# robertknight/rten

Hardware: NVIDIA H100
Metric: resnet50_fp32_inferences_per_sec (higher is better)
Workload: dtype f32(tf32 mma, explicit opt-in)

## Files before the change

rten_b200/csrc/umma_gemm.cu:

```cuda
#include <cuda.h>
#include <cuda_runtime.h>

#include <algorithm>
#include <array>
#include <cmath>
#include <vector>
#include <cmath>
#include <cstdint>
#include <cstdio>
#include <cstdlib>

#include "math.cuh"
#include "ptx.cuh"
#include "rowops.h"
#include "umma_gemm.h"
#include "umma_kernel.cuh"

namespace rtb {

typedef CUresult (*EncodeTiledFn)(CUtensorMap*, CUtensorMapDataType, cuuint32_t, void*, const cuuint64_t*,
                                  const cuuint64_t*, const cuuint32_t*, const cuuint32_t*, CUtensorMapInterleave,
                                  CUtensorMapSwizzle, CUtensorMapL2promotion, CUtensorMapFloatOOBfill);

static EncodeTiledFn get_encode(rten_ctx* ctx) {
    if (!ctx->encode_tiled) {
        void* fn = nullptr;
        cudaDriverEntryPointQueryResult qres;
        if (cudaGetDriverEntryPoint("cuTensorMapEncodeTiled", &fn, cudaEnableDefault, &qres) != cudaSuccess ||
            qres != cudaDriverEntryPointSuccess)
            return nullptr;
        ctx->encode_tiled = fn;
    }
    return reinterpret_cast<EncodeTiledFn>(ctx->encode_tiled);
}

bool tma_compatible(const OperandDesc& od, int esize, int rank) {
    if (reinterpret_cast<uintptr_t>(od.base) & 15) return false;
    if (od.strides[0] != 1) return false;
    for (int i = 1; i < rank; i++) {
        if (od.dims[i] > 1) {
            if ((od.strides[i] * esize) % 16 != 0) return false;
            if (od.strides[i] * esize >= (1ll << 40)) return false;
        }
    }
    for (int i = 0; i < rank; i++)
        if (od.dims[i] < 1 || od.dims[i] > 0xFFFFFFFFll) return false;
    return true;
}

bool encode_map(rten_ctx* ctx, CUtensorMap* map, const OperandDesc& od, int esize, bool is_f32,
                const uint32_t box[4], const uint32_t estr[4]) {
    EncodeTiledFn enc = get_encode(ctx);
    if (!enc) return false;
    cuuint64_t dims[4];
    cuuint64_t strides[3];
    cuuint32_t b[4], es[4];
    for (int i = 0; i < 4; i++) {
        dims[i] = (cuuint64_t)od.dims[i];
        b[i] = box[i];
        es[i] = estr[i];
    }
    for (int i = 1; i < 4; i++) {
        long long s = od.strides[i] * esize;
        if (s == 0 || od.dims[i] == 1) s = 16;
        strides[i - 1] = (cuuint64_t)s;
    }
    CUresult r = enc(map, is_f32 ? CU_TENSOR_MAP_DATA_TYPE_FLOAT32 : CU_TENSOR_MAP_DATA_TYPE_UINT8, 4,
                     const_cast<void*>(od.base), dims, strides, b, es, CU_TENSOR_MAP_INTERLEAVE_NONE,
                     CU_TENSOR_MAP_SWIZZLE_128B, CU_TENSOR_MAP_L2_PROMOTION_L2_256B,
                     CU_TENSOR_MAP_FLOAT_OOB_FILL_NONE);
    return r == CUDA_SUCCESS;
}

static void pick_conv_tile(const ConvGeom& g, int& tw, int& th, int& tb) {
    double best = -1.0;
    tw = th = tb = 1;
    for (int w = 1; w <= std::min(g.OW, 128); w++) {
        if (w * g.sx > 256) break;
        for (int h = 1; h <= std::min(g.OH, 128 / w); h++) {
            if (h * g.sy > 256) break;
            int b = std::min(g.B, 128 / (w * h));
            if (b < 1) continue;
            long long tiles = (long long)((g.OW + w - 1) / w) * ((g.OH + h - 1) / h) * ((g.B + b - 1) / b);
            double eff = (double)g.B * g.OH * g.OW / ((double)tiles * 128.0);
            if (eff > best + 1e-9 || (eff > best - 1e-9 && w > tw)) {
                best = eff;
                tw = w;
                th = h;
                tb = b;
            }
        }
    }
}

struct Plan {
    int bn = 32, splitk = 1, nbuf = 1;
};

struct Prepared {
    KParams p;
    uint32_t abox[4], aes[4], bbox_k;
    uint32_t a_rows;
    long long batch;
    OperandDesc od, ord;
    uint32_t dbox[4];
    int tma_store, res_tma;
    int wide;
    int step;
    int esize, kelems;
};

constexpr int SK_CNT_INTS = 1 << 16;
static int smem_budget_for(int n_stg) { return 227 * 1024 - SMEM_FIXED_BYTES - n_stg * STG_BYTES; }
static int wide_stages(int stage_bytes) { return std::min(MAX_STAGES, (227 * 1024 - WIDE_SMEM_FIXED_BYTES) / stage_bytes); }
static bool is_wide(int bn) { return bn > ACC_STRIDE; }

static Epi pick_epilogue(const GemmLaunch& L, int tma_store, int res_tma, int splitk) {
    const EpilogueDesc& e = L.epi;
    auto aligned = [](const void* ptr) { return (reinterpret_cast<uintptr_t>(ptr) & 15) == 0; };
    bool fast = tma_store && (L.N % 32) == 0 && !getenv("RTEN_B200_NO_FAST") && e.bias_kind != 2 &&
                (e.r == nullptr || res_tma) && (e.bias_kind != 1 || aligned(e.bias));
    if (L.kind == 1)
        fast = fast && (!(e.za || e.za8) || aligned(e.colsum)) && (!e.zb || e.zb_len == 1 || (e.zb_len == L.N && aligned(e.zb))) &&
               (!e.scale || e.scale_len == 1 || (e.scale_len == L.N && aligned(e.scale)));
    if (!fast) return Epi::Generic;
    const bool gelu = e.act > 1;
    if (!getenv("RTEN_B200_NO_PLAIN") && e.act <= 3) {
        if (L.kind == 0 && e.alpha == 1.0f && !e.range && (e.r == nullptr || e.r_scale == 1.0f))
            return gelu ? Epi::PlainF32Gelu : Epi::PlainF32;
        if (L.kind == 1 && e.scale && !e.za && !e.zb && (e.scale_len == 1 || e.scale_len == L.N) && splitk == 1 &&
            (!e.za8 || e.colsum))
            return gelu ? Epi::PlainI8Gelu : Epi::PlainI8;
    }
    return gelu ? Epi::FastGelu : Epi::Fast;
}

static const char* epi_name(Epi v) {
    static const char* const names[] = {"Generic", "Fast", "FastGelu", "PlainF32", "PlainF32Gelu", "PlainI8", "PlainI8Gelu"};
    return names[(int)v];
}

static bool is_plain_f32(Epi v) { return v == Epi::PlainF32 || v == Epi::PlainF32Gelu; }

struct PlanShape {
    long long tiles_n, units_m, tiles, units;
    int kb_per, stage_bytes, stages, n_stg;
};

static bool plan_shape(const Prepared& q, const Plan& pl, PlanShape& ps) {
    const KParams& p = q.p;
    if (is_wide(pl.bn)) {
        if ((pl.bn != 128 && pl.bn != 256) || !q.wide || pl.splitk != 1) return false;
        if (pl.bn == 256 && q.p.epi.act > 1) return false;
    } else if (pl.bn < 16 || pl.bn % 32 || pl.bn % q.step) {
        return false;
    }
    if (pl.nbuf < (q.res_tma ? 2 : 1) || pl.nbuf > 4) return false;
    ps.tiles_n = (p.N + pl.bn - 1) / pl.bn;
    ps.units_m = p.tiles_m;
    ps.tiles = ps.units_m * ps.tiles_n * q.batch;
    ps.units = ps.tiles * pl.splitk;
    if (ps.units > 0x7FFFFFFFll) return false;
    ps.kb_per = (p.k_blocks + pl.splitk - 1) / pl.splitk;
    if (pl.splitk > 1) {
        if (pl.bn % 32 || (long long)(pl.splitk - 1) * ps.kb_per >= p.k_blocks) return false;
        if (ps.tiles * 2 > SK_CNT_INTS) return false;
    }
    ps.n_stg = 2 * pl.nbuf;
    ps.stage_bytes = A_STAGE_BYTES + pl.bn * KBYTES;
    ps.stages = is_wide(pl.bn) ? wide_stages(ps.stage_bytes) : std::min(MAX_STAGES, smem_budget_for(ps.n_stg) / ps.stage_bytes);
    if (ps.stages < 2) return false;
    return true;
}

static double plan_cost(const Prepared& q, const Plan& pl, const PlanShape& ps, int num_sms) {
    const double active = (double)std::min<long long>(ps.units, num_sms);
    const double waves = std::ceil((double)ps.units / num_sms);
    const double bw = std::min(64.0, 7400.0 / active);
    const double mmas = 4.0;
    const double t_kb = std::max(mmas * std::max(42.0, (double)pl.bn), ps.stage_bytes / bw);
    double t_stage = std::max(t_kb, 320.0 + mmas * 42.0);
    t_stage = std::max(t_stage, 2300.0 / ps.stages);
    const double mainloop = ps.kb_per * t_stage;
    const double epi = is_wide(pl.bn) ? (pl.bn / 32.0) * 400.0 + 600.0 : (pl.bn / 32.0) * 350.0 / 2.0 + 600.0;
    double unit = (is_wide(pl.bn) ? mainloop + epi : std::max(mainloop, epi)) + 1500.0;
    double cost = waves * unit + 2500.0;
    if (pl.splitk > 1) cost += epi * (1.0 + 0.25 * pl.splitk) + 1500.0;

    return cost;
}

static void enumerate_plans(const Prepared& q, int num_sms, std::vector<std::pair<double, Plan>>& out) {
    const KParams& p = q.p;
    const int nmax = (p.N + q.step - 1) / q.step * q.step;
    static const int splits[] = {1, 2, 3, 4, 5, 6, 8, 10, 12, 16};
    for (int bn : {32, 64, 128, 256}) {
        if (bn > nmax && bn != 32) break;
        for (int sk : splits) {
            Plan pl;
            pl.bn = bn;
            pl.splitk = sk;
            if (sk > 1 && p.k_blocks / sk < 4) continue;
            const int kb_per = (p.k_blocks + sk - 1) / sk;
            pl.nbuf = (q.res_tma || kb_per < 24) ? 2 : 1;
            PlanShape ps;
            if (is_wide(bn)) {
                pl.nbuf = 2;
            } else if (pl.nbuf == 2 && !getenv("RTEN_B200_NO_NBUF3")) {
                PlanShape ps2;
                const bool ok2 = plan_shape(q, pl, ps2);
                pl.nbuf = 3;
                if (!plan_shape(q, pl, ps) || (ps.stages < 3 && !(ok2 && ps.stages == ps2.stages))) pl.nbuf = 2;
            }
            if (!plan_shape(q, pl, ps)) continue;
            if (sk > 1 && ps.tiles >= 2 * num_sms) continue;
            if (ps.stages < 2) continue;
            out.emplace_back(plan_cost(q, pl, ps, num_sms), pl);
        }
    }
    std::sort(out.begin(), out.end(), [](const std::pair<double, Plan>& x, const std::pair<double, Plan>& y) {
        return x.first < y.first;
    });
}

static rten_status prepare_launch(rten_ctx* ctx, const GemmLaunch& L, Prepared& q) {
    const int esize = L.kind == 0 ? 4 : 1;
    const int kelems = KBYTES / esize;
    if (!tma_compatible(L.a, esize, 4) || !tma_compatible(L.b, esize, 4)) return RTEN_ERR_UNSUPPORTED_VALUE;
    if (L.M <= 0 || L.N <= 0 || L.K <= 0) return RTEN_ERR_UNSUPPORTED_VALUE;
    q.esize = esize;
    q.kelems = kelems;
    KParams& p = q.p;
    memset(&p, 0, sizeof(p));
    p.M = L.M;
    p.N = L.N;
    p.K = L.K;
    p.z0 = L.z0;
    p.z1 = L.z1;
    p.kelems = kelems;
    p.conv = L.conv;
    p.epi = L.epi;
    p.c_blocks = 1;
    p.kw = 1;
    for (int i = 0; i < 4; i++) q.aes[i] = 1;
    if (L.conv) {
        const ConvGeom& g = L.g;
        pick_conv_tile(g, p.tw, p.th, p.tb);
        p.tiles_x = (g.OW + p.tw - 1) / p.tw;
        p.tiles_y = (g.OH + p.th - 1) / p.th;
        int tiles_b = (g.B + p.tb - 1) / p.tb;
        p.tiles_m = p.tiles_x * p.tiles_y * tiles_b;
        p.OH = g.OH;
        p.OW = g.OW;
        p.Bn = g.B;
        p.sy = g.sy;
        p.sx = g.sx;
        p.dy = g.dy;
        p.dx = g.dx;
        p.pt = g.pt;
        p.pl = g.pl;
        p.kw = g.kw;
        p.c_blocks = (g.C + kelems - 1) / kelems;
        p.k_blocks = g.kh * g.kw * p.c_blocks;
        p.z0 = p.z1 = 1;
        q.abox[0] = kelems;
        q.abox[1] = p.tw * g.sx;
        q.abox[2] = p.th * g.sy;
        q.abox[3] = p.tb;
        q.aes[1] = g.sx;
        q.aes[2] = g.sy;
        q.a_rows = p.tw * p.th * p.tb;
        q.batch = 1;
    } else {
        p.tiles_m = (L.M + BM - 1) / BM;
        p.k_blocks = (L.K + kelems - 1) / kelems;
        q.abox[0] = kelems;
        q.abox[1] = BM;
        q.abox[2] = 1;
        q.abox[3] = 1;
        q.a_rows = BM;
        q.batch = (long long)L.z0 * L.z1;
        p.a_bcast0 = (L.a.dims[2] == 1 && L.z0 > 1) ? 1 : 0;
        p.a_bcast1 = (L.a.dims[3] == 1 && L.z1 > 1) ? 1 : 0;
        p.b_bcast0 = (L.b.dims[2] == 1 && L.z0 > 1) ? 1 : 0;
        p.b_bcast1 = (L.b.dims[3] == 1 && L.z1 > 1) ? 1 : 0;
    }
    OperandDesc& od = q.od;
    OperandDesc& ord = q.ord;
    q.dbox[0] = 32;
    q.dbox[1] = q.dbox[2] = q.dbox[3] = 1;
    const EpilogueDesc& e = L.epi;
    od.base = e.d;
    od.dims[0] = L.N;
    od.strides[0] = 1;
    if (L.conv) {
        od.dims[1] = L.g.OW;
        od.dims[2] = L.g.OH;
        od.dims[3] = L.g.B;
        od.strides[1] = e.s_z1;
        od.strides[2] = e.s_row;
        od.strides[3] = e.s_z0;
        q.dbox[1] = p.tw;
        q.dbox[2] = p.th;
        q.dbox[3] = p.tb;
    } else {
        od.dims[1] = L.M;
        od.dims[2] = L.z0;
        od.dims[3] = L.z1;
        od.strides[1] = e.s_row;
        od.strides[2] = e.s_z0;
        od.strides[3] = e.s_z1;
        q.dbox[1] = BM;
    }
    q.tma_store = (e.s_col == 1 && L.N >= 4 && tma_compatible(od, 4, 4)) ? 1 : 0;
    if (getenv("RTEN_B200_NO_TMA_STORE")) q.tma_store = 0;
    ord = od;
    ord.base = e.r;
    if (L.conv) {
        ord.strides[1] = e.r_z1;
        ord.strides[2] = e.r_row;
        ord.strides[3] = e.r_z0;
    } else {
        ord.strides[1] = e.r_row;
        ord.strides[2] = e.r_z0;
        ord.strides[3] = e.r_z1;
    }
    q.res_tma = (q.tma_store && (L.kind == 0 || e.scale) && e.r && e.r_col == 1 && (L.N % 32) == 0 &&
                 (e.bias_kind != 1 || (reinterpret_cast<uintptr_t>(e.bias) & 15) == 0) && tma_compatible(ord, 4, 4))
                    ? 1
                    : 0;
    for (int i = 1; i < 4; i++)
        if (ord.dims[i] > 1 && ord.strides[i] == 0) q.res_tma = 0;
    if (getenv("RTEN_B200_NO_RES_TMA")) q.res_tma = 0;
    p.res_tx_bytes = q.a_rows * KBYTES;
    q.step = q.tma_store ? 32 : 16;
    q.wide = is_plain_f32(pick_epilogue(L, q.tma_store, q.res_tma, 1)) && !getenv("RTEN_B200_NO_WIDE");
    return RTEN_OK;
}

static size_t splitk_ws_bytes(const PlanShape& ps, const Plan& pl) {
    return pl.splitk > 1 ? (size_t)ps.tiles * pl.splitk * (pl.bn / 32) * 4096 * 4 : 0;
}

static rten_status ensure_splitk_counters(rten_ctx* ctx) {
    if (!ctx->sk_counters) {
        cudaError_t ce = cudaMalloc(&ctx->sk_counters, SK_CNT_INTS * sizeof(int));
        if (ce != cudaSuccess) return fail_cuda(ctx, ce, "split-K counters");
        ce = cudaMemset(ctx->sk_counters, 0, SK_CNT_INTS * sizeof(int));
        if (ce != cudaSuccess) return fail_cuda(ctx, ce, "split-K counters");
    }
    return RTEN_OK;
}

static rten_status launch_plan(rten_ctx* ctx, const GemmLaunch& L, const Prepared& q, const Plan& pl, bool verbose,
                               void* ws = nullptr) {
    PlanShape ps;
    if (!plan_shape(q, pl, ps)) return RTEN_ERR_UNSUPPORTED_VALUE;
    KParams p = q.p;
    p.bn = pl.bn;
    p.splitk = pl.splitk;
    p.nbuf = pl.nbuf;
    p.tma_store = q.tma_store;
    p.res_tma = q.res_tma ? 1 : 0;
    p.kb_per = ps.kb_per;
    p.tiles_n = (int)ps.tiles_n;
    p.tiles_total = (int)ps.tiles;
    p.units_total = (int)ps.units;
    p.d_tiles_n.set(p.tiles_n);
    p.d_tiles_m.set(p.tiles_m);
    p.d_z0.set(p.z0);
    p.d_tiles_x.set(p.conv ? p.tiles_x : 1);
    p.d_tiles_y.set(p.conv ? p.tiles_y : 1);
    p.d_tiles_total.set(p.tiles_total);
    p.d_c_blocks.set(p.c_blocks);
    p.d_kw.set(p.kw);
    p.d_tw.set(p.conv ? p.tw : 1);
    p.d_th.set(p.conv ? p.th : 1);
    p.stage_bytes = ps.stage_bytes;
    p.tx_bytes = q.a_rows * KBYTES + p.bn * KBYTES;
    p.stages = ps.stages;
    p.sgn = L.kind == 0 ? 0 : (L.a_signed ? 1 : 0) | (L.b_signed ? 2 : 0);
    if (p.splitk > 1) {
        RTB_TRY(ensure_splitk_counters(ctx));
        if (!ws) RTB_TRY(temp_alloc(ctx, splitk_ws_bytes(ps, pl), &ws));
        p.sk_ws = reinterpret_cast<uint32_t*>(ws);
        p.sk_cnt = reinterpret_cast<int*>(ctx->sk_counters);
    }

    uint32_t bbox[4] = {(uint32_t)q.kelems, (uint32_t)p.bn, 1, 1}, bes[4] = {1, 1, 1, 1}, des[4] = {1, 1, 1, 1};
    CUtensorMap map_a, map_b;
    if (!encode_map(ctx, &map_a, L.a, q.esize, L.kind == 0, q.abox, q.aes)) return RTEN_ERR_UNSUPPORTED_VALUE;
    if (!encode_map(ctx, &map_b, L.b, q.esize, L.kind == 0, bbox, bes)) return RTEN_ERR_UNSUPPORTED_VALUE;
    CUtensorMap map_d = map_a, map_r = map_a, map_a2 = map_a;
    p.x3_cb = L.x3_cb;
    if (L.x3_cb && !encode_map(ctx, &map_a2, L.a_lo, q.esize, true, q.abox, q.aes)) return RTEN_ERR_UNSUPPORTED_VALUE;
    if (p.tma_store && !encode_map(ctx, &map_d, q.od, 4, true, q.dbox, des)) {
        p.tma_store = 0;
        p.res_tma = 0;
        map_d = map_a;
    }
    if (p.res_tma && !encode_map(ctx, &map_r, q.ord, 4, true, q.dbox, des)) {
        p.res_tma = 0;
        map_r = map_a;
    }
    const Epi epi = pick_epilogue(L, p.tma_store, p.res_tma, p.splitk);
    if (epi == Epi::Generic && (L.kind == 1 || L.epi.act > 1)) p.res_tma = 0;

    if (verbose)
        fprintf(stderr, "[umma_gemm] kind=%d conv=%d M=%d N=%d K=%d kb=%d tiles_m=%d bn=%d splitk=%d units=%d stages=%d tma_store=%d res_tma=%d nbuf=%d box=%dx%dx%d epi=%s\n",
                L.kind, L.conv, L.M, L.N, L.K, p.k_blocks, p.tiles_m, p.bn, p.splitk, p.units_total, p.stages, p.tma_store,
                p.res_tma, p.nbuf, p.tw, p.th, p.tb, epi_name(epi));
    if (is_wide(p.bn) && !is_plain_f32(epi)) return RTEN_ERR_UNSUPPORTED_VALUE;
    const size_t smem_bytes = (size_t)p.stages * p.stage_bytes +
                              (is_wide(p.bn) ? WIDE_SMEM_FIXED_BYTES : ps.n_stg * STG_BYTES + SMEM_FIXED_BYTES);
    using Kernel = void (*)(CUtensorMap, CUtensorMap, CUtensorMap, CUtensorMap, CUtensorMap, KParams);
    static const Kernel narrow[2][7] = {
        {umma_gemm_kernel<0, Epi::Generic>, umma_gemm_kernel<0, Epi::Fast>, umma_gemm_kernel<0, Epi::FastGelu>,
         umma_gemm_kernel<0, Epi::PlainF32>, umma_gemm_kernel<0, Epi::PlainF32Gelu>, nullptr, nullptr},
        {umma_gemm_kernel<1, Epi::Generic>, umma_gemm_kernel<1, Epi::Fast>, umma_gemm_kernel<1, Epi::FastGelu>, nullptr,
         nullptr, umma_gemm_kernel<1, Epi::PlainI8>, umma_gemm_kernel<1, Epi::PlainI8Gelu>}};
    const Kernel kern = !is_wide(p.bn)              ? narrow[L.kind][(int)epi]
                        : epi == Epi::PlainF32Gelu ? umma_wide_kernel<Epi::PlainF32Gelu>
                                                   : umma_wide_kernel<Epi::PlainF32>;

    cudaLaunchConfig_t cfg;
    memset(&cfg, 0, sizeof(cfg));
    cfg.gridDim = dim3(std::min(p.units_total, ctx->num_sms));
    cfg.blockDim = dim3(is_wide(p.bn) ? WIDE_THREADS : NUM_THREADS);
    cfg.dynamicSmemBytes = smem_bytes;
    cfg.stream = ctx->stream;
    cudaLaunchAttribute attr[1];
    attr[0].id = cudaLaunchAttributeProgrammaticStreamSerialization;
    attr[0].val.programmaticStreamSerializationAllowed = 1;
    cfg.attrs = attr;
    cfg.numAttrs = getenv("RTEN_B200_NO_PDL") ? 0 : 1;
    cudaError_t e = cudaFuncSetAttribute(kern, cudaFuncAttributeMaxDynamicSharedMemorySize, 227 * 1024);
    if (e == cudaSuccess) e = cudaLaunchKernelEx(&cfg, kern, map_a, map_b, map_d, map_r, map_a2, p);
    if (e != cudaSuccess) return fail_cuda(ctx, e, "umma_gemm launch");
    e = cudaGetLastError();
    if (e != cudaSuccess) return fail_cuda(ctx, e, "umma_gemm launch");
    count_launch(ctx);
    return RTEN_OK;
}

static std::vector<long long> tune_key(const GemmLaunch& L, const Prepared& q) {
    const EpilogueDesc& e = L.epi;
    std::vector<long long> k = {L.kind, L.conv, L.M, L.N, L.K, L.z0, L.z1, q.tma_store, q.res_tma, e.act, e.bias_kind,
                                e.r != nullptr, (e.za != nullptr || e.za8 != nullptr), e.zb != nullptr, e.scale != nullptr,
                                L.a.strides[1], L.b.strides[1], L.x3_cb};
    if (L.conv) {
        const ConvGeom& g = L.g;
        for (long long v : {g.B, g.H, g.W, g.C, g.OH, g.OW, g.kh, g.kw, g.sy, g.sx, g.dy, g.dx, g.pt, g.pl}) k.push_back(v);
    }
    return k;
}

static Plan plan_from_array(const std::array<int, 3>& a) {
    Plan pl;
    pl.bn = a[0];
    pl.splitk = a[1];
    pl.nbuf = a[2];
    return pl;
}

static rten_status launch_tf32x3(rten_ctx* ctx, const GemmLaunch& L0) {
    GemmLaunch L = L0;
    const long long d0 = L0.a.dims[0];
    const long long d0p = (d0 + 3) / 4 * 4;
    auto split = [&](const OperandDesc& src, OperandDesc& dst, int role, void* into) -> rten_status {
        const long long planes = role == 2 ? 1 : 3;
        long long dims[4], strides[4], n = planes * d0p;
        for (int i = 0; i < 4; i++) {
            dims[i] = (i > 0 && src.strides[i] == 0) ? 1 : src.dims[i];
            strides[i] = src.strides[i];
        }
        for (int i = 1; i < 4; i++) n *= dims[i];
        void* buf = into;
        if (!buf) RTB_TRY(temp_alloc(ctx, (size_t)n * 4, &buf));
        RTB_TRY(launch_tf32x3_split(ctx, (const float*)src.base, (float*)buf, dims, strides, d0p, role));
        dst = src;
        dst.base = buf;
        dst.dims[0] = planes * d0p;
        long long st = planes * d0p;
        for (int i = 1; i < 4; i++) {
            dst.strides[i] = (src.strides[i] == 0 && src.dims[i] > 1) ? 0 : st;
            st *= dims[i];
        }
        return RTEN_OK;
    };
    if (L0.b.dims[0] != d0) return RTEN_ERR_UNSUPPORTED_VALUE;
    if (L0.b_x3_slot && !getenv("RTEN_B200_X3_NO_CACHE")) {
        if (!*L0.b_x3_slot && !ctx->capturing) {
            long long n = 3 * d0p;
            for (int i = 1; i < 4; i++) n *= (L0.b.strides[i] == 0 ? 1 : L0.b.dims[i]);
            void* buf = nullptr;
            if (cudaMalloc(&buf, (size_t)n * 4) != cudaSuccess) return fail(ctx, RTEN_ERR_CUDA, "cudaMalloc failed for the 3xTF32 copy of a prepacked operand");
            OperandDesc tmp;
            const rten_status st = split(L0.b, tmp, 1, buf);
            if (st != RTEN_OK) {
                cudaFree(buf);
                return st;
            }
            *L0.b_x3_slot = buf;
        }
    }
    if (L0.b_x3_slot && *L0.b_x3_slot && !getenv("RTEN_B200_X3_NO_CACHE")) {
        L.b = L0.b;
        L.b.base = *L0.b_x3_slot;
        L.b.dims[0] = 3 * d0p;
        long long st = 3 * d0p;
        for (int i = 1; i < 4; i++) {
            const long long di = L0.b.strides[i] == 0 ? 1 : L0.b.dims[i];
            L.b.strides[i] = (L0.b.strides[i] == 0 && L0.b.dims[i] > 1) ? 0 : st;
            st *= di;
        }
    } else {
        RTB_TRY(split(L0.b, L.b, 1, nullptr));
    }
    const bool two_plane = d0 % 32 == 0 && tma_compatible(L0.a, 4, 4) && !getenv("RTEN_B200_X3_THREE_PLANES");
    if (two_plane && L0.a_lo_base) {
        L.a_lo = L0.a;
        L.a_lo.base = L0.a_lo_base;
        L.x3_cb = (int)(d0 / 32);
    } else if (two_plane) {
        RTB_TRY(split(L0.a, L.a_lo, 2, nullptr));
        L.x3_cb = (int)(d0 / 32);
    } else {
        RTB_TRY(split(L0.a, L.a, 0, nullptr));
    }
    if (L.conv)
        L.g.C = (int)(3 * d0p);
    L.K = L.conv ? (int)(L0.K / d0 * 3 * d0p) : (int)(3 * d0p);
    L.b_x3_slot = nullptr;
    L.a_lo_base = nullptr;
    const int saved = ctx->f32_mode;
    ctx->f32_mode = RTEN_F32_TF32;
    const rten_status st = launch_umma_gemm(ctx, L);
    ctx->f32_mode = saved;
    return st;
}

rten_status launch_umma_gemm(rten_ctx* ctx, const GemmLaunch& L) {
    if (L.kind == 0 && ctx->f32_mode == RTEN_F32_TF32X3) return launch_tf32x3(ctx, L);
    if (L.conv && L.kind == 0 && L.g.kh * L.g.kw > 1 && !L.x3_cb) {
        const rten_status hs = launch_umma_halo_conv(ctx, L);
        if (hs != RTEN_ERR_UNSUPPORTED_VALUE) return hs;
    }
    Prepared q;
    RTB_TRY(prepare_launch(ctx, L, q));
    const bool verbose = getenv("RTEN_B200_VERBOSE") != nullptr;
    const bool forced = getenv("RTEN_B200_FORCE_BN") || getenv("RTEN_B200_FORCE_SPLITK");
    if (!forced && !ctx->tune_cache.empty()) {
        auto hit = ctx->tune_cache.find(tune_key(L, q));
        if (hit != ctx->tune_cache.end()) {
            PlanShape ps;
            if (hit->second[0] < 0) {
                const rten_status hs = launch_umma_halo_conv(ctx, L, hit->second[1], hit->second[2]);
                if (hs != RTEN_ERR_UNSUPPORTED_VALUE) return hs;
            } else
            if (plan_shape(q, plan_from_array(hit->second), ps)) return launch_plan(ctx, L, q, plan_from_array(hit->second), verbose);
            if (verbose) fprintf(stderr, "[umma_gemm] recorded plan no longer valid for this problem: re-planning\n");
            ctx->tune_cache.erase(hit);
        }
    }
    std::vector<std::pair<double, Plan>> cands;
    enumerate_plans(q, ctx->num_sms, cands);
    if (cands.empty()) return RTEN_ERR_UNSUPPORTED_VALUE;
    Plan plan = cands[0].second;

    if (forced) {
        const char* fb = getenv("RTEN_B200_FORCE_BN");
        const char* fs = getenv("RTEN_B200_FORCE_SPLITK");
        bool found = false;
        for (const auto& c : cands) {
            const Plan& x = c.second;
            if (fb && x.bn != atoi(fb)) continue;
// ... 124 lines not shown
```

rten_b200/csrc/umma_kernel.cuh:

```cuda
#pragma once
#include <cuda.h>
#include <cuda_runtime.h>

#include <cstdint>

#include "math.cuh"
#include "ptx.cuh"
#include "umma_gemm.h"

namespace rtb {

constexpr int BM = 128;
constexpr int KBYTES = 128;
constexpr int A_STAGE_BYTES = BM * KBYTES;
constexpr int ACC_STRIDE = 64;
constexpr int PRODUCER_WARP = 12;
constexpr int NUM_THREADS = 416;
constexpr int STG_BYTES = 128 * 128;
constexpr int MAX_STAGES = 8;

struct FastDiv {
    uint32_t d = 1, mul = 0, shr = 0;
    __host__ void set(int div) {
        d = (uint32_t)(div < 1 ? 1 : div);
        if (d == 1) {
            mul = 0;
            shr = 0;
            return;
        }
        uint32_t lg = 0;
        while ((1ull << lg) < d) lg++;
        const uint32_t p = 31 + lg;
        mul = (uint32_t)(((1ull << p) + d - 1) / d);
        shr = p - 32;
    }
    __device__ __forceinline__ int div(int n) const { return d == 1 ? n : (int)(__umulhi((uint32_t)n, mul) >> shr); }
    __device__ __forceinline__ void divmod(int n, int& q, int& r) const {
        q = div(n);
        r = n - q * (int)d;
    }
};

enum class Epi { Generic, Fast, FastGelu, PlainF32, PlainF32Gelu, PlainI8, PlainI8Gelu };

struct KParams {
    int M, N, K, z0, z1;
    int tiles_m, tiles_n, tiles_total;
    int k_blocks, kelems;
    int bn, stages;
    uint32_t stage_bytes, tx_bytes;
    int sgn;
    int conv;
    int tw, th, tb, tiles_x, tiles_y;
    int OH, OW, Bn;
    int sy, sx, dy, dx, pt, pl, kw, c_blocks;
    int a_bcast0, a_bcast1, b_bcast0, b_bcast1;
    int nbuf;
    int res_tma;
    uint32_t res_tx_bytes;
    int tma_store;
    int splitk;
    int kb_per;
    int units_total;
    int x3_cb;
    FastDiv d_tiles_n, d_tiles_m, d_z0, d_tiles_x, d_tiles_y, d_tiles_total, d_c_blocks, d_kw, d_tw, d_th;
    uint32_t* sk_ws;
    int* sk_cnt;
    EpilogueDesc epi;
};

struct TileCoord {
    int n0;
    int m0;
    int z0, z1;
    int ox0, oy0, b0;
};

__device__ __forceinline__ TileCoord decode_tile(const KParams& p, int t) {
    TileCoord c;
    int n_blk, rest, m_blk, z;
    p.d_tiles_n.divmod(t, rest, n_blk);
    p.d_tiles_m.divmod(rest, z, m_blk);
    c.n0 = n_blk * p.bn;
    c.m0 = m_blk * BM;
    p.d_z0.divmod(z, c.z1, c.z0);
    c.ox0 = c.oy0 = c.b0 = 0;
    if (p.conv) {
        int xt, r2, yt, bt;
        p.d_tiles_x.divmod(m_blk, r2, xt);
        p.d_tiles_y.divmod(r2, bt, yt);
        c.ox0 = xt * p.tw;
        c.oy0 = yt * p.th;
        c.b0 = bt * p.tb;
    }
    return c;
}

__device__ __forceinline__ int4 out_coord(const KParams& p, const TileCoord& tc, int col) {
    return p.conv ? make_int4(tc.n0 + col, tc.ox0, tc.oy0, tc.b0) : make_int4(tc.n0 + col, tc.m0, tc.z0, tc.z1);
}

__device__ __forceinline__ void plain_f32_pair(uint32_t& v0, uint32_t& v1, bool res, float2 rr, float2 bb, bool relu) {
    if (res) add_f32x2(v0, v1, rr.x, rr.y);
    add_f32x2(v0, v1, bb.x, bb.y);
    if (relu) {
        v0 = __float_as_uint(fmaxf(__uint_as_float(v0), 0.0f));
        v1 = __float_as_uint(fmaxf(__uint_as_float(v1), 0.0f));
    }
}

__device__ __forceinline__ void bulk_wait_read(int n) {
    switch (n) {
        case 0: asm volatile("cp.async.bulk.wait_group.read 0;" ::: "memory"); break;
        case 1: asm volatile("cp.async.bulk.wait_group.read 1;" ::: "memory"); break;
        case 2: asm volatile("cp.async.bulk.wait_group.read 2;" ::: "memory"); break;
        default: asm volatile("cp.async.bulk.wait_group.read 3;" ::: "memory"); break;
    }
}

__device__ __forceinline__ int f32_to_ordered(float f) {
    const int i = __float_as_int(f);
    return i >= 0 ? i : i ^ 0x7fffffff;
}
__device__ __forceinline__ void range_commit(int* range, float lo, float hi) {
#pragma unroll
    for (int o = 16; o > 0; o >>= 1) {
        lo = fminf(lo, __shfl_xor_sync(0xffffffffu, lo, o));
        hi = fmaxf(hi, __shfl_xor_sync(0xffffffffu, hi, o));
    }
    if ((threadIdx.x & 31) == 0 && lo <= hi) {
        atomicMin(&range[0], f32_to_ordered(lo));
        atomicMax(&range[1], f32_to_ordered(hi));
    }
}

__device__ __noinline__ float4 act4(float4 x, int act) {
    if (act == 2) {
        gelu_ref_x2(x.x, x.y);
        gelu_ref_x2(x.z, x.w);
        return x;
    }
    x.x = apply_act(x.x, act);
    x.y = apply_act(x.y, act);
    x.z = apply_act(x.z, act);
    x.w = apply_act(x.w, act);
    return x;
}

__device__ __forceinline__ bool splitk_publish(const KParams& p, int t, int ks, int grp, int q, int lane, uint32_t t_acc,
                                               int* flag, uint32_t acc_smem) {
    const int r = q * 32 + lane;
    const int nchunks = p.bn >> 5;
    for (int c0 = grp * 32; c0 < p.bn; c0 += 64) {
        uint32_t v[32];
        acc_ld(acc_smem, t_acc + c0, v);
        uint32_t* w = p.sk_ws + ((((size_t)t * p.splitk + ks) * nchunks + (c0 >> 5)) << 12) + r;
#pragma unroll
        for (int j = 0; j < 32; j++) __stcg(w + j * 128, v[j]);
    }
    __threadfence();
    asm volatile("bar.sync %0, 128;" ::"r"(1 + grp) : "memory");
    if (q == 0 && lane == 0) {
        int* cnt = p.sk_cnt + t * 2 + grp;
        const int old = atomicAdd(cnt, 1);
        const int last = old == p.splitk - 1;
        if (last) *cnt = 0;
        __threadfence();
        *flag = last;
    }
    asm volatile("bar.sync %0, 128;" ::"r"(1 + grp) : "memory");
    return *reinterpret_cast<volatile int*>(flag) != 0;
}

template <int KIND>
__device__ __forceinline__ void splitk_sum(const KParams& p, int t, int c0, int r, uint32_t (&v)[32]) {
    const int nchunks = p.bn >> 5;
    const uint32_t* w = p.sk_ws + ((((size_t)t * p.splitk) * nchunks + (c0 >> 5)) << 12) + r;
    const size_t stride = (size_t)nchunks << 12;
#pragma unroll
    for (int j = 0; j < 32; j++) v[j] = __ldcg(w + j * 128);
#pragma unroll 1
    for (int s = 1; s < p.splitk; s++) {
        w += stride;
#pragma unroll
        for (int j = 0; j < 32; j++) {
            const uint32_t x = __ldcg(w + j * 128);
            if (KIND == 0)
                v[j] = __float_as_uint(__fadd_rn(__uint_as_float(v[j]), __uint_as_float(x)));
            else
                v[j] += x;
        }
    }
}

struct SmemLayout {
    uint8_t* smem;
    uint64_t *full_bar, *empty_bar, *acc_full, *acc_empty, *res_bar;
    int* sk_flag;
    float* bias;
    uint32_t acc_smem;
};

}

#include "umma_epilogue.cuh"

namespace rtb {

template <int KIND, int SGN, int N>
__device__ __forceinline__ void mma_units(const KParams& p, const SmemLayout& L, int worker, int n_workers) {
    const int lane = threadIdx.x & 31;
    const uint32_t smem0 = smem_u32(L.smem);
    uint32_t ring = 0, aphase = 0;
    int stage = 0;
    for (int u = worker, it = 0; u < p.units_total; u += n_workers, it++) {
        const int kb0 = p.d_tiles_total.div(u) * p.kb_per, kb1 = min(p.k_blocks, kb0 + p.kb_per);
        const int acc = it & 1;
        acc_t<KIND> d0[N / 2], d1[N / 2];
#pragma unroll
        for (int i = 0; i < N / 2; i++) d0[i] = d1[i] = 0;
        int prev = -1;
        for (int kb = kb0; kb < kb1; kb++) {
            mbar_wait(&L.full_bar[stage], (ring >> stage) & 1);
            wgmma_fence_operand(d0);
            wgmma_fence_operand(d1);
            wgmma_fence();
            const uint32_t sa = smem0 + stage * p.stage_bytes;
            const uint64_t adesc = make_kmajor_sw128_desc(sa);
            const uint64_t bdesc = make_kmajor_sw128_desc(sa + A_STAGE_BYTES);
#pragma unroll
            for (int k = 0; k < 4; k++) {
                wgmma_k<KIND, SGN, N>(d0, adesc + 2 * k, bdesc + 2 * k);
                wgmma_k<KIND, SGN, N>(d1, adesc + (64 * KBYTES >> 4) + 2 * k, bdesc + 2 * k);
            }
            wgmma_commit();
            wgmma_fence_operand(d0);
            wgmma_fence_operand(d1);
            wgmma_wait<1>();
            if (prev >= 0 && lane == 0) mbar_arrive(&L.empty_bar[prev]);
            prev = stage;
            ring ^= 1u << stage;
            if (++stage == p.stages) stage = 0;
        }
        wgmma_wait<0>();
        wgmma_fence_operand(d0);
        wgmma_fence_operand(d1);
        if (prev >= 0 && lane == 0) mbar_arrive(&L.empty_bar[prev]);
        mbar_wait(&L.acc_empty[acc], ((aphase >> acc) & 1) ^ 1);
        aphase ^= 1u << acc;
        acc_store_frag<N>(L.acc_smem, d0, 0, acc * ACC_STRIDE);
        acc_store_frag<N>(L.acc_smem, d1, 64, acc * ACC_STRIDE);
        mbar_arrive(&L.acc_full[acc]);
    }
}

template <int KIND, int N>
__device__ __forceinline__ void mma_role(const KParams& p, const SmemLayout& L, int worker, int n_workers) {
    if (KIND == 0) mma_units<KIND, 0, N>(p, L, worker, n_workers);
    else if (p.sgn == 0) mma_units<KIND, 0, N>(p, L, worker, n_workers);
    else if (p.sgn == 1) mma_units<KIND, 1, N>(p, L, worker, n_workers);
    else if (p.sgn == 2) mma_units<KIND, 2, N>(p, L, worker, n_workers);
    else mma_units<KIND, 3, N>(p, L, worker, n_workers);
}

__device__ __forceinline__ void producer_role(const KParams& p, const CUtensorMap* tma_a, const CUtensorMap* tma_a2,
                                              const CUtensorMap* tma_b, const SmemLayout& L, int worker, int n_workers) {
    uint8_t* smem = L.smem;
    uint64_t* empty_bar = L.empty_bar;
    uint32_t ring = 0;
    int stage = 0;
    const uint32_t smem0 = smem_u32(smem);
    const uint32_t full0 = smem_u32(L.full_bar);
    for (int u = worker; u < p.units_total; u += n_workers) {
        int t, ks;
        p.d_tiles_total.divmod(u, ks, t);
        const int kb0 = ks * p.kb_per, kb1 = min(p.k_blocks, kb0 + p.kb_per);
        const TileCoord tc = decode_tile(p, t);
        int tap, cb, ky, kx;
        p.d_c_blocks.divmod(kb0, tap, cb);
        p.d_kw.divmod(tap, ky, kx);
        int seg = 0, sblk = p.conv ? cb : kb0;
        if (p.x3_cb)
            while (sblk >= p.x3_cb) {
                sblk -= p.x3_cb;
                seg++;
            }
        if (u == worker) asm volatile("griddepcontrol.wait;" ::: "memory");
        for (int kb = kb0; kb < kb1; kb++) {
            mbar_wait(&empty_bar[stage], ((ring >> stage) & 1) ^ 1);
            if (elect_one()) {
                const uint32_t fb = full0 + stage * 8;
                mbar_expect_tx_u32(fb, p.tx_bytes);
                const uint32_t sa = smem0 + stage * p.stage_bytes;
                const uint32_t sb = sa + A_STAGE_BYTES;
                const CUtensorMap* ma = (p.x3_cb && seg == 0) ? tma_a2 : tma_a;
                if (p.conv) {
                    const int c0 = cb * p.kelems;
                    const int ca = p.x3_cb ? sblk * p.kelems : c0;
                    tma_load_4d_u32(sa, ma, fb, ca, tc.ox0 * p.sx - p.pl + kx * p.dx, tc.oy0 * p.sy - p.pt + ky * p.dy, tc.b0);
                    tma_load_4d_u32(sb, tma_b, fb, c0, tc.n0, tap, 0);
                } else {
                    const int k0 = kb * p.kelems;
                    const int ka = p.x3_cb ? sblk * p.kelems : k0;
                    tma_load_4d_u32(sa, ma, fb, ka, tc.m0, p.a_bcast0 ? 0 : tc.z0, p.a_bcast1 ? 0 : tc.z1);
                    tma_load_4d_u32(sb, tma_b, fb, k0, tc.n0, p.b_bcast0 ? 0 : tc.z0, p.b_bcast1 ? 0 : tc.z1);
                }
            }
            if (p.x3_cb && ++sblk == p.x3_cb) {
                sblk = 0;
                seg = seg == 2 ? 0 : seg + 1;
            }
            if (++cb == p.c_blocks) {
                cb = 0;
                tap++;
                if (++kx == p.kw) {
                    kx = 0;
                    ky++;
                }
            }
            __syncwarp();
            ring ^= 1u << stage;
            if (++stage == p.stages) stage = 0;
        }
    }
}

constexpr int SMEM_FIXED_BYTES = 1024  + 4096  + ACC_SMEM_BYTES;
static_assert(ACC_SMEM_BYTES % 1024 == 0, "operand stages must stay 1024-B aligned");
static_assert(2 * ACC_STRIDE <= ACC_COLS, "two accumulator stages");

__device__ __forceinline__ SmemLayout carve_smem(uint8_t* smem_raw) {
    uint8_t* base = reinterpret_cast<uint8_t*>((reinterpret_cast<uintptr_t>(smem_raw) + 1023) & ~uintptr_t(1023));
    SmemLayout L;
    L.full_bar = reinterpret_cast<uint64_t*>(base);
    L.empty_bar = L.full_bar + MAX_STAGES;
    L.acc_full = L.empty_bar + MAX_STAGES;
    L.acc_empty = L.acc_full + 2;
    L.res_bar = L.acc_empty + 2;
    L.sk_flag = reinterpret_cast<int*>(L.res_bar + 8) + 2;
    L.bias = reinterpret_cast<float*>(base + 1024);
    L.acc_smem = smem_u32(base + 4096);
    L.smem = base + 4096 + ACC_SMEM_BYTES;
    return L;
}

__device__ __forceinline__ void kernel_setup(const SmemLayout& L) {
    const int warp = threadIdx.x >> 5;
    const int lane = threadIdx.x & 31;
    if (warp == PRODUCER_WARP) {
        if (lane < MAX_STAGES) {
            mbar_init(&L.full_bar[lane], 1);
            mbar_init(&L.empty_bar[lane], 4);
        }
        fence_mbar_init();
        __syncwarp();
        asm volatile("bar.arrive 15, %0;" ::"r"(NUM_THREADS) : "memory");
        return;
    }
    if (warp == 1) {
        if (lane < 2)
            mbar_init(&L.acc_full[lane], 128);
        else if (lane < 4)
            mbar_init(&L.acc_empty[lane - 2], 8);
        else if (lane < 12)
            mbar_init(&L.res_bar[lane - 4], 1);
        fence_mbar_init();
    }
    asm volatile("bar.sync 15, %0;" ::"r"(NUM_THREADS) : "memory");
}

template <int KIND, Epi E>
__global__ void __launch_bounds__(NUM_THREADS, 1)
umma_gemm_kernel(const __grid_constant__ CUtensorMap tma_a, const __grid_constant__ CUtensorMap tma_b,
                 const __grid_constant__ CUtensorMap tma_d, const __grid_constant__ CUtensorMap tma_r,
                 const __grid_constant__ CUtensorMap tma_a2, const __grid_constant__ KParams p) {
    extern __shared__ uint8_t smem_raw[];
    const SmemLayout L = carve_smem(smem_raw);
    if (threadIdx.x == 0) {
        tma_prefetch_desc(&tma_a);
        tma_prefetch_desc(&tma_b);
        if (p.tma_store) tma_prefetch_desc(&tma_d);
        if (p.res_tma) tma_prefetch_desc(&tma_r);
        if (p.x3_cb) tma_prefetch_desc(&tma_a2);
    }
    kernel_setup(L);
    if (threadIdx.x >> 5 != PRODUCER_WARP) asm volatile("griddepcontrol.wait;" ::: "memory");
    asm volatile("griddepcontrol.launch_dependents;" ::: "memory");
    const int worker = (int)blockIdx.x, n_workers = (int)gridDim.x;
    const int warp = threadIdx.x >> 5;
    if (warp == PRODUCER_WARP) {
        producer_role(p, &tma_a, &tma_a2, &tma_b, L, worker, n_workers);
    } else if (warp < 4) {
        if (p.bn == 32)
            mma_role<KIND, 32>(p, L, worker, n_workers);
        else
            mma_role<KIND, 64>(p, L, worker, n_workers);
    } else {
        epilogue<KIND, E>(p, L, &tma_d, &tma_r, worker, n_workers);
    }
}

constexpr int WIDE_THREADS = 384;
constexpr int WIDE_SMEM_FIXED_BYTES = 1024 + 2 * STG_BYTES + 2048;

template <int N>
__device__ __forceinline__ void wgmma_wide(float (&d)[N / 2], uint64_t adesc, uint64_t bdesc) {
    if constexpr (N == 128) wgmma_tf32_n128(d, adesc, bdesc);
    else wgmma_tf32_n256(d, adesc, bdesc);
}

__device__ __forceinline__ void consumers_sync() { asm volatile("bar.sync 1, 256;" ::: "memory"); }

__device__ __forceinline__ SmemLayout carve_wide_smem(uint8_t* smem_raw, const KParams& p) {
    uint8_t* base = reinterpret_cast<uint8_t*>((reinterpret_cast<uintptr_t>(smem_raw) + 1023) & ~uintptr_t(1023));
    uint8_t* tail = base + (size_t)p.stages * p.stage_bytes + 2 * STG_BYTES;
    SmemLayout L;
    L.smem = base;
    L.full_bar = reinterpret_cast<uint64_t*>(tail);
    L.empty_bar = L.full_bar + MAX_STAGES;
    L.res_bar = L.empty_bar + MAX_STAGES;
    L.acc_full = L.acc_empty = nullptr;
    L.sk_flag = nullptr;
    L.bias = reinterpret_cast<float*>(tail + 256);
    L.acc_smem = 0;
    return L;
}

template <Epi E, int N>
__device__ __forceinline__ void wide_consumer(const KParams& p, const SmemLayout& L, const CUtensorMap* tma_d,
                                              const CUtensorMap* tma_r, int worker, int n_workers) {
    const int t = threadIdx.x - 128;
    const int wg = t >> 7;
    const int lane = threadIdx.x & 31;
    const int row0 = 64 * wg + 16 * ((t & 127) >> 5) + (lane >> 2);
    const int sw = lane >> 2;
    const int cq = lane & 3;
    const bool issuer = t == 0;
    const EpilogueDesc& e = p.epi;
    const uint32_t smem0 = smem_u32(L.smem);
    uint8_t* const stg0 = L.smem + (size_t)p.stages * p.stage_bytes;
    float* const bias_s = L.bias;
    uint32_t ring = 0, rphase = 0;
    uint32_t ci = 0;
    int stage = 0;
    auto load_residual = [&](const TileCoord& tc, int c0, int buf) {
        uint64_t* rb = &L.res_bar[buf];
        mbar_expect_tx(rb, p.res_tx_bytes);
        const int4 x = out_coord(p, tc, c0);
        tma_load_4d(stg0 + buf * STG_BYTES, tma_r, rb, x.x, x.y, x.z, x.w);
    };
    for (int u = worker; u < p.units_total; u += n_workers) {
        {
            const TileCoord tc = decode_tile(p, u);
            if (t < N) bias_s[t] = (e.bias_kind == 1 && tc.n0 + t < p.N) ? __ldg(e.bias + tc.n0 + t) : 0.0f;
            if (issuer) {
                bulk_wait_read(0);
                if (p.res_tma) load_residual(tc, 0, ci & 1);
            }
        }
        float d[N / 2];
#pragma unroll
        for (int i = 0; i < N / 2; i++) d[i] = 0.0f;
        int prev = -1;
        for (int kb = 0; kb < p.k_blocks; kb++) {
            mbar_wait(&L.full_bar[stage], (ring >> stage) & 1);
            wgmma_fence_operand(d);
            wgmma_fence();
            const uint32_t sa = smem0 + stage * p.stage_bytes;
            const uint64_t adesc = make_kmajor_sw128_desc(sa + wg * (64 * KBYTES));
            const uint64_t bdesc = make_kmajor_sw128_desc(sa + A_STAGE_BYTES);
#pragma unroll
            for (int k = 0; k < 4; k++) wgmma_wide<N>(d, adesc + 2 * k, bdesc + 2 * k);
            wgmma_commit();
            wgmma_fence_operand(d);
            wgmma_wait<1>();
            if (prev >= 0 && lane == 0) mbar_arrive(&L.empty_bar[prev]);
            prev = stage;
            ring ^= 1u << stage;
            if (++stage == p.stages) stage = 0;
        }
        wgmma_wait<0>();
        wgmma_fence_operand(d);
        if (prev >= 0 && lane == 0) mbar_arrive(&L.empty_bar[prev]);
        const TileCoord tc = decode_tile(p, u);
        consumers_sync();
#pragma unroll
        for (int k = 0; k < N / 32; k++, ci++) {
            const int buf = ci & 1;
            uint8_t* stg = stg0 + buf * STG_BYTES;
            const int nbase = tc.n0 + 32 * k;
            if (issuer) {
                bulk_wait_read(0);
                if (p.res_tma && k + 1 < N / 32) load_residual(tc, 32 * (k + 1), buf ^ 1);
            }
            if (p.res_tma) {
                mbar_wait(&L.res_bar[buf], (rphase >> buf) & 1);
                rphase ^= 1u << buf;
            }
#pragma unroll
            for (int j = 0; j < 4; j++) {
                const int i0 = 16 * k + 4 * j;
                float2* px[2];
#pragma unroll
                for (int h = 0; h < 2; h++)
                    px[h] = reinterpret_cast<float2*>(stg + (row0 + 8 * h) * 128 + (((2 * j + (cq >> 1)) ^ sw) << 4) + 8 * (cq & 1));
                if (nbase < p.N) {
                    const float2 bb = *reinterpret_cast<const float2*>(bias_s + 32 * k + 8 * j + 2 * cq);
#pragma unroll
                    for (int h = 0; h < 2; h++) {
                        uint32_t v0 = __float_as_uint(d[i0 + 2 * h]), v1 = __float_as_uint(d[i0 + 2 * h + 1]);
                        float2 rr = make_float2(0.f, 0.f);
                        if (p.res_tma) rr = *px[h];
                        plain_f32_pair(v0, v1, p.res_tma, rr, bb, e.act == 1);
                        d[i0 + 2 * h] = __uint_as_float(v0);
                        d[i0 + 2 * h + 1] = __uint_as_float(v1);
                    }
                    if (E == Epi::PlainF32Gelu) {
                        const float4 g = act4(make_float4(d[i0], d[i0 + 1], d[i0 + 2], d[i0 + 3]), e.act);
                        d[i0] = g.x;
                        d[i0 + 1] = g.y;
                        d[i0 + 2] = g.z;
                        d[i0 + 3] = g.w;
                    }
                }
#pragma unroll
                for (int h = 0; h < 2; h++) *px[h] = make_float2(d[i0 + 2 * h], d[i0 + 2 * h + 1]);
            }
            fence_proxy_async();
            consumers_sync();
            if (issuer) {
                const int4 x = out_coord(p, tc, 32 * k);
                tma_store_4d(tma_d, stg, x.x, x.y, x.z, x.w);
                asm volatile("cp.async.bulk.commit_group;" ::: "memory");
            }
        }
    }
    if (issuer) asm volatile("cp.async.bulk.wait_group.read 0;" ::: "memory");
}

template <Epi E>
__global__ void __launch_bounds__(WIDE_THREADS, 1)
umma_wide_kernel(const __grid_constant__ CUtensorMap tma_a, const __grid_constant__ CUtensorMap tma_b,
                 const __grid_constant__ CUtensorMap tma_d, const __grid_constant__ CUtensorMap tma_r,
                 const __grid_constant__ CUtensorMap tma_a2, const __grid_constant__ KParams p) {
    extern __shared__ uint8_t smem_raw[];
    const SmemLayout L = carve_wide_smem(smem_raw, p);
    const int warp = threadIdx.x >> 5;
    const int lane = threadIdx.x & 31;
    if (threadIdx.x == 0) {
        tma_prefetch_desc(&tma_a);
        tma_prefetch_desc(&tma_b);
        tma_prefetch_desc(&tma_d);
        if (p.res_tma) tma_prefetch_desc(&tma_r);
        if (p.x3_cb) tma_prefetch_desc(&tma_a2);
    }
    if (warp == 1) {
        if (lane < MAX_STAGES) {
            mbar_init(&L.full_bar[lane], 1);
            mbar_init(&L.empty_bar[lane], 8);
        } else if (lane < MAX_STAGES + 2) {
            mbar_init(&L.res_bar[lane - MAX_STAGES], 1);
        }
        fence_mbar_init();
    }
    __syncthreads();
    if (warp >= 4) asm volatile("griddepcontrol.wait;" ::: "memory");
    asm volatile("griddepcontrol.launch_dependents;" ::: "memory");
    if (warp < 4) {
        asm volatile("setmaxnreg.dec.sync.aligned.u32 56;");
        if (warp == 0) producer_role(p, &tma_a, &tma_a2, &tma_b, L, (int)blockIdx.x, (int)gridDim.x);
    } else {
        asm volatile("setmaxnreg.inc.sync.aligned.u32 224;");
        if (E == Epi::PlainF32Gelu || p.bn == 128)
            wide_consumer<E, 128>(p, L, &tma_d, &tma_r, (int)blockIdx.x, (int)gridDim.x);
        else
            wide_consumer<E, 256>(p, L, &tma_d, &tma_r, (int)blockIdx.x, (int)gridDim.x);
    }
}

}
```

Before: 14110.

## Add split-K support to the wide (bn=128) WGMMA GEMM kernel

Lets the wide warp-specialized kernel run with split-K at bn=128. Units are decoded so that the K-slices of one tile are adjacent, and each slice writes its partial accumulator to a global workspace. The last-arriving CTA, found through an atomic counter, sums the partials and runs the fused epilogue. A cost-model branch lets the planner choose these plans, which is meant to fill more SMs on small-M, large-K layers. The cost is extra workspace traffic, an atomic and fence handshake per tile, and a 32MB workspace cap.

```diff
diff --git a/rten_b200/csrc/umma_gemm.cu b/rten_b200/csrc/umma_gemm.cu
--- a/rten_b200/csrc/umma_gemm.cu
+++ b/rten_b200/csrc/umma_gemm.cu
@@ -106,6 +106,7 @@
     uint32_t dbox[4];
     int tma_store, res_tma;
     int wide;
+    int wide_splitk;
     int step;
     int esize, kelems;
 };
@@ -114,6 +115,7 @@
 static int smem_budget_for(int n_stg) { return 227 * 1024 - SMEM_FIXED_BYTES - n_stg * STG_BYTES; }
 static int wide_stages(int stage_bytes) { return std::min(MAX_STAGES, (227 * 1024 - WIDE_SMEM_FIXED_BYTES) / stage_bytes); }
 static bool is_wide(int bn) { return bn > ACC_STRIDE; }
+constexpr size_t WIDE_SK_WS_MAX = 32u << 20;
 
 static Epi pick_epilogue(const GemmLaunch& L, int tma_store, int res_tma, int splitk) {
     const EpilogueDesc& e = L.epi;
@@ -147,11 +149,15 @@
     int kb_per, stage_bytes, stages, n_stg;
 };
 
+static size_t splitk_ws_bytes(const PlanShape& ps, const Plan& pl) {
+    return pl.splitk > 1 ? (size_t)ps.tiles * pl.splitk * (pl.bn / 32) * 4096 * 4 : 0;
+}
+
 static bool plan_shape(const Prepared& q, const Plan& pl, PlanShape& ps) {
     const KParams& p = q.p;
     if (is_wide(pl.bn)) {
-        if ((pl.bn != 128 && pl.bn != 256) || !q.wide || pl.splitk != 1) return false;
-        if (pl.bn == 256 && q.p.epi.act > 1) return false;
+        if ((pl.bn != 128 && pl.bn != 256) || !q.wide || (pl.splitk != 1 && !q.wide_splitk)) return false;
+        if (pl.bn == 256 && (q.p.epi.act > 1 || pl.splitk > 1)) return false;
     } else if (pl.bn < 16 || pl.bn % 32 || pl.bn % q.step) {
         return false;
     }
@@ -165,6 +171,7 @@
     if (pl.splitk > 1) {
         if (pl.bn % 32 || (long long)(pl.splitk - 1) * ps.kb_per >= p.k_blocks) return false;
         if (ps.tiles * 2 > SK_CNT_INTS) return false;
+        if (is_wide(pl.bn) && splitk_ws_bytes(ps, pl) > WIDE_SK_WS_MAX) return false;
     }
     ps.n_stg = 2 * pl.nbuf;
     ps.stage_bytes = A_STAGE_BYTES + pl.bn * KBYTES;
@@ -183,6 +190,10 @@
     t_stage = std::max(t_stage, 2300.0 / ps.stages);
     const double mainloop = ps.kb_per * t_stage;
     const double epi = is_wide(pl.bn) ? (pl.bn / 32.0) * 400.0 + 600.0 : (pl.bn / 32.0) * 350.0 / 2.0 + 600.0;
+    if (is_wide(pl.bn) && pl.splitk > 1) {
+        const double part = 128.0 * pl.bn * 4.0 / bw;
+        return waves * (mainloop + part + 1500.0) + std::ceil((double)ps.tiles / num_sms) * (pl.splitk * part + epi) + 2500.0;
+    }
     double unit = (is_wide(pl.bn) ? mainloop + epi : std::max(mainloop, epi)) + 1500.0;
     double cost = waves * unit + 2500.0;
     if (pl.splitk > 1) cost += epi * (1.0 + 0.25 * pl.splitk) + 1500.0;
@@ -335,11 +346,8 @@
     p.res_tx_bytes = q.a_rows * KBYTES;
     q.step = q.tma_store ? 32 : 16;
     q.wide = is_plain_f32(pick_epilogue(L, q.tma_store, q.res_tma, 1)) && !getenv("RTEN_B200_NO_WIDE");
+    q.wide_splitk = q.wide && !getenv("RTEN_B200_NO_WIDE_SPLITK");
     return RTEN_OK;
-}
-
-static size_t splitk_ws_bytes(const PlanShape& ps, const Plan& pl) {
-    return pl.splitk > 1 ? (size_t)ps.tiles * pl.splitk * (pl.bn / 32) * 4096 * 4 : 0;
 }
 
 static rten_status ensure_splitk_counters(rten_ctx* ctx) {
@@ -372,6 +380,7 @@
     p.d_tiles_x.set(p.conv ? p.tiles_x : 1);
     p.d_tiles_y.set(p.conv ? p.tiles_y : 1);
     p.d_tiles_total.set(p.tiles_total);
+    p.d_splitk.set(p.splitk);
     p.d_c_blocks.set(p.c_blocks);
     p.d_kw.set(p.kw);
     p.d_tw.set(p.conv ? p.tw : 1);
@@ -419,9 +428,9 @@
          umma_gemm_kernel<0, Epi::PlainF32>, umma_gemm_kernel<0, Epi::PlainF32Gelu>, nullptr, nullptr},
         {umma_gemm_kernel<1, Epi::Generic>, umma_gemm_kernel<1, Epi::Fast>, umma_gemm_kernel<1, Epi::FastGelu>, nullptr,
          nullptr, umma_gemm_kernel<1, Epi::PlainI8>, umma_gemm_kernel<1, Epi::PlainI8Gelu>}};
-    const Kernel kern = !is_wide(p.bn)              ? narrow[L.kind][(int)epi]
-                        : epi == Epi::PlainF32Gelu ? umma_wide_kernel<Epi::PlainF32Gelu>
-                                                   : umma_wide_kernel<Epi::PlainF32>;
+    static const Kernel wide[2][2] = {{umma_wide_kernel<Epi::PlainF32, false>, umma_wide_kernel<Epi::PlainF32Gelu, false>},
+                                      {umma_wide_kernel<Epi::PlainF32, true>, umma_wide_kernel<Epi::PlainF32Gelu, true>}};
+    const Kernel kern = !is_wide(p.bn) ? narrow[L.kind][(int)epi] : wide[p.splitk > 1][epi == Epi::PlainF32Gelu];
 
     cudaLaunchConfig_t cfg;
     memset(&cfg, 0, sizeof(cfg));
diff --git a/rten_b200/csrc/umma_kernel.cuh b/rten_b200/csrc/umma_kernel.cuh
--- a/rten_b200/csrc/umma_kernel.cuh
+++ b/rten_b200/csrc/umma_kernel.cuh
@@ -63,7 +63,7 @@
     int kb_per;
     int units_total;
     int x3_cb;
-    FastDiv d_tiles_n, d_tiles_m, d_z0, d_tiles_x, d_tiles_y, d_tiles_total, d_c_blocks, d_kw, d_tw, d_th;
+    FastDiv d_tiles_n, d_tiles_m, d_z0, d_tiles_x, d_tiles_y, d_tiles_total, d_c_blocks, d_kw, d_tw, d_th, d_splitk;
     uint32_t* sk_ws;
     int* sk_cnt;
     EpilogueDesc epi;
@@ -96,6 +96,13 @@
     return c;
 }
 
+__device__ __forceinline__ void decode_unit(const KParams& p, int u, int& ks, int& t) {
+    if (p.bn > ACC_STRIDE)
+        p.d_splitk.divmod(u, t, ks);
+    else
+        p.d_tiles_total.divmod(u, ks, t);
+}
+
 __device__ __forceinline__ int4 out_coord(const KParams& p, const TileCoord& tc, int col) {
     return p.conv ? make_int4(tc.n0 + col, tc.ox0, tc.oy0, tc.b0) : make_int4(tc.n0 + col, tc.m0, tc.z0, tc.z1);
 }
@@ -273,7 +280,7 @@
     const uint32_t full0 = smem_u32(L.full_bar);
     for (int u = worker; u < p.units_total; u += n_workers) {
         int t, ks;
-        p.d_tiles_total.divmod(u, ks, t);
+        decode_unit(p, u, ks, t);
         const int kb0 = ks * p.kb_per, kb1 = min(p.k_blocks, kb0 + p.kb_per);
         const TileCoord tc = decode_tile(p, t);
         int tap, cb, ky, kx;
@@ -420,13 +427,54 @@
     L.empty_bar = L.full_bar + MAX_STAGES;
     L.res_bar = L.empty_bar + MAX_STAGES;
     L.acc_full = L.acc_empty = nullptr;
-    L.sk_flag = nullptr;
+    L.sk_flag = reinterpret_cast<int*>(tail + 192);
     L.bias = reinterpret_cast<float*>(tail + 256);
     L.acc_smem = 0;
     return L;
 }
 
-template <Epi E, int N>
+template <int N>
+__device__ __forceinline__ bool wide_splitk(const KParams& p, int tile, int ks, int t, float (&d)[N / 2], int* flag) {
+    constexpr int PART = N / 8 * 256;
+    const float4* ws = reinterpret_cast<const float4*>(p.sk_ws) + (size_t)tile * p.splitk * PART + t;
+    float4* mine = const_cast<float4*>(ws) + ks * PART;
+#pragma unroll
+    for (int i = 0; i < N / 8; i++) __stcg(mine + i * 256, make_float4(d[4 * i], d[4 * i + 1], d[4 * i + 2], d[4 * i + 3]));
+    __threadfence();
+    consumers_sync();
+    if (t == 0) {
+        int* cnt = p.sk_cnt + tile * 2;
+        const int last = atomicAdd(cnt, 1) == p.splitk - 1;
+        if (last) *cnt = 0;
+        __threadfence();
+        *flag = last;
+    }
+    consumers_sync();
+    if (*reinterpret_cast<volatile int*>(flag) == 0) return false;
+#pragma unroll
+    for (int i = 0; i < N / 8; i++) {
+        const float4 x = __ldcg(ws + i * 256);
+        d[4 * i] = x.x;
+        d[4 * i + 1] = x.y;
+        d[4 * i + 2] = x.z;
+        d[4 * i + 3] = x.w;
+    }
+#pragma unroll 1
+    for (int s = 1; s < p.splitk; s++) {
+        ws += PART;
+#pragma unroll
+        for (int i = 0; i < N / 8; i++) {
+            const float4 x = __ldcg(ws + i * 256);
+            d[4 * i] = __fadd_rn(d[4 * i], x.x);
+            d[4 * i + 1] = __fadd_rn(d[4 * i + 1], x.y);
+            d[4 * i + 2] = __fadd_rn(d[4 * i + 2], x.z);
+            d[4 * i + 3] = __fadd_rn(d[4 * i + 3], x.w);
+        }
+    }
+    return true;
+}
+
+template <Epi E, int N, bool SPLIT>
 __device__ __forceinline__ void wide_consumer(const KParams& p, const SmemLayout& L, const CUtensorMap* tma_d,
                                               const CUtensorMap* tma_r, int worker, int n_workers) {
     const int t = threadIdx.x - 128;
@@ -450,19 +498,23 @@
         tma_load_4d(stg0 + buf * STG_BYTES, tma_r, rb, x.x, x.y, x.z, x.w);
     };
     for (int u = worker; u < p.units_total; u += n_workers) {
+        int nkb;
         {
-            const TileCoord tc = decode_tile(p, u);
+            int tile = u, ks = 0;
+            if (SPLIT) decode_unit(p, u, ks, tile);
+            nkb = min(p.kb_per, p.k_blocks - ks * p.kb_per);
+            const TileCoord tc = decode_tile(p, tile);
             if (t < N) bias_s[t] = (e.bias_kind == 1 && tc.n0 + t < p.N) ? __ldg(e.bias + tc.n0 + t) : 0.0f;
             if (issuer) {
                 bulk_wait_read(0);
-                if (p.res_tma) load_residual(tc, 0, ci & 1);
+                if (p.res_tma && !SPLIT) load_residual(tc, 0, ci & 1);
             }
         }
         float d[N / 2];
 #pragma unroll
         for (int i = 0; i < N / 2; i++) d[i] = 0.0f;
         int prev = -1;
-        for (int kb = 0; kb < p.k_blocks; kb++) {
+        for (; nkb > 0; nkb--) {
             mbar_wait(&L.full_bar[stage], (ring >> stage) & 1);
             wgmma_fence_operand(d);
             wgmma_fence();
@@ -482,7 +534,13 @@
         wgmma_wait<0>();
         wgmma_fence_operand(d);
         if (prev >= 0 && lane == 0) mbar_arrive(&L.empty_bar[prev]);
-        const TileCoord tc = decode_tile(p, u);
+        int tile = u;
+        if constexpr (SPLIT) {
+            int ks;
+            decode_unit(p, u, ks, tile);
+            if (!wide_splitk<N>(p, tile, ks, t, d, L.sk_flag)) continue;
+        }
+        const TileCoord tc = decode_tile(p, tile);
         consumers_sync();
 #pragma unroll
         for (int k = 0; k < N / 32; k++, ci++) {
@@ -491,6 +549,7 @@
             const int nbase = tc.n0 + 32 * k;
             if (issuer) {
                 bulk_wait_read(0);
+                if (SPLIT && p.res_tma && k == 0) load_residual(tc, 0, buf);
                 if (p.res_tma && k + 1 < N / 32) load_residual(tc, 32 * (k + 1), buf ^ 1);
             }
             if (p.res_tma) {
@@ -538,7 +597,7 @@
     if (issuer) asm volatile("cp.async.bulk.wait_group.read 0;" ::: "memory");
 }
 
-template <Epi E>
+template <Epi E, bool SPLIT>
 __global__ void __launch_bounds__(WIDE_THREADS, 1)
 umma_wide_kernel(const __grid_constant__ CUtensorMap tma_a, const __grid_constant__ CUtensorMap tma_b,
                  const __grid_constant__ CUtensorMap tma_d, const __grid_constant__ CUtensorMap tma_r,
@@ -571,11 +630,13 @@
         if (warp == 0) producer_role(p, &tma_a, &tma_a2, &tma_b, L, (int)blockIdx.x, (int)gridDim.x);
     } else {
         asm volatile("setmaxnreg.inc.sync.aligned.u32 224;");
-        if (E == Epi::PlainF32Gelu || p.bn == 128)
-            wide_consumer<E, 128>(p, L, &tma_d, &tma_r, (int)blockIdx.x, (int)gridDim.x);
+        if constexpr (SPLIT)
+            wide_consumer<E, 128, true>(p, L, &tma_d, &tma_r, (int)blockIdx.x, (int)gridDim.x);
+        else if (E == Epi::PlainF32Gelu || p.bn == 128)
+            wide_consumer<E, 128, false>(p, L, &tma_d, &tma_r, (int)blockIdx.x, (int)gridDim.x);
         else
-            wide_consumer<E, 256>(p, L, &tma_d, &tma_r, (int)blockIdx.x, (int)gridDim.x);
-    }
-}
-
-}
+            wide_consumer<E, 256, false>(p, L, &tma_d, &tma_r, (int)blockIdx.x, (int)gridDim.x);
+    }
+}
+
+}
```

Measured after the change: 14300 (median of 6 runs). +1.3%, better.
